# wavey-ai/soundkit

Measured on AMD Instinct MI355X. Metric: AAC-LC 1024-sample frames/s (whole node) + xrealtime, batch=4096 48 kHz stereo, higher is better.
Workload: dtype f32 (synthesis f32; s16 between the kernels as in the reference; FIR: the 16-bit samples as 2 x f16 exactly, the f32 taps as 2 x f16 to 2^-24, f32 accumulate; 1.0e-7 rel. RMS vs f64)

## Files before the change

### soundkit_amd/csrc/aac_synth.hip

```cpp
#include "sk_device.h"

#define SK_SYNTH_LOAD(p) (*(p))
#define SK_SYNTH_STORE(v, p) (*(p) = (v))

namespace sk {

namespace {

typedef float f2 __attribute__((ext_vector_type(2)));
typedef float f4 __attribute__((ext_vector_type(4)));

#ifndef SK_SYNTH_BLOCK_WAVES
#define SK_SYNTH_BLOCK_WAVES 4
#endif
constexpr int kWavesPerBlock = SK_SYNTH_BLOCK_WAVES;
#ifndef SK_WAVES_PER_SIMD
#define SK_WAVES_PER_SIMD 3
#endif
#ifndef SK_PREFETCH_DEPTH
#define SK_PREFETCH_DEPTH 1
#endif
constexpr int kDepth = SK_PREFETCH_DEPTH;
constexpr int kWavesPerSimd = SK_WAVES_PER_SIMD;
#ifndef SK_SYNTH_HOLD_ONE
#define SK_SYNTH_HOLD_ONE 1
#endif
constexpr int kExchange = 576;
constexpr int kStage = 1024;

__device__ __forceinline__ f2 cmul(f2 a, f2 b) {
    return (f2){fmaf(a.x, b.x, -a.y * b.y), fmaf(a.x, b.y, a.y * b.x)};
}
__device__ __forceinline__ f2 cadd(f2 a, f2 b) { return (f2){a.x + b.x, a.y + b.y}; }
__device__ __forceinline__ f2 csub(f2 a, f2 b) { return (f2){a.x - b.x, a.y - b.y}; }
__device__ __forceinline__ f2 mul_mi(f2 a) { return (f2){a.y, -a.x}; }

__device__ __forceinline__ void dft8(f2 (&x)[8]) {
    const float h = 0.70710678118654752440f;
    f2 t0 = cadd(x[0], x[4]), t1 = csub(x[0], x[4]);
    f2 t2 = cadd(x[2], x[6]), t3 = mul_mi(csub(x[2], x[6]));
    f2 e0 = cadd(t0, t2), e2 = csub(t0, t2), e1 = cadd(t1, t3), e3 = csub(t1, t3);
    f2 u0 = cadd(x[1], x[5]), u1 = csub(x[1], x[5]);
    f2 u2 = cadd(x[3], x[7]), u3 = mul_mi(csub(x[3], x[7]));
    f2 o0 = cadd(u0, u2), o2 = csub(u0, u2), o1 = cadd(u1, u3), o3 = csub(u1, u3);
    f2 w1 = (f2){(o1.x + o1.y) * h, (o1.y - o1.x) * h};
    f2 w2 = mul_mi(o2);
    f2 w3 = (f2){(o3.y - o3.x) * h, -(o3.x + o3.y) * h};
    x[0] = cadd(e0, o0); x[4] = csub(e0, o0);
    x[1] = cadd(e1, w1); x[5] = csub(e1, w1);
    x[2] = cadd(e2, w2); x[6] = csub(e2, w2);
    x[3] = cadd(e3, w3); x[7] = csub(e3, w3);
}

__device__ __forceinline__ void wave_sync() {
    __builtin_amdgcn_fence(__ATOMIC_ACQ_REL, "wavefront");
    __builtin_amdgcn_wave_barrier();
}

typedef const __attribute__((address_space(4))) SynthEntry *const_entries;
__device__ __forceinline__ const_entries as_constant(const SynthEntry *p) {
    return reinterpret_cast<const_entries>(reinterpret_cast<uintptr_t>(p));
}

typedef uint32_t u2 __attribute__((ext_vector_type(2)));
__device__ __forceinline__ u2 pack4_s16(const f4 &v) {
    return (u2){dev_pack2_s16(v.x, v.y), dev_pack2_s16(v.z, v.w)};
}

__device__ __forceinline__ const float *first_half_window(const float *win, int seq, int prev_shape) {
    return seq == 3 ? win + 6656 + 1024 * prev_shape : win + 2048 * prev_shape;
}
__device__ __forceinline__ const float *second_half_window(const float *win, int seq, int shape) {
    return seq == 1 ? win + 4608 + 1024 * shape : win + 2048 * shape + 1024;
}
// ... 2 lines not shown
typedef __attribute__((address_space(3))) f4 lds_f4;
typedef __attribute__((address_space(3))) float lds_f;

__device__ __forceinline__ void read_positions(const lds_f *buf, int lane, float (&v)[16]) {
#pragma unroll
    for (int r = 0; r < 2; ++r) {
        const int j = 4 * lane + 256 * r;
        const f4 f = *reinterpret_cast<const lds_f4 *>(buf + j);
        const f4 m = *reinterpret_cast<const lds_f4 *>(buf + 1020 - j);
        v[8 * r + 0] = f.x; v[8 * r + 1] = f.y; v[8 * r + 2] = f.z; v[8 * r + 3] = f.w;
        v[8 * r + 4] = m.x; v[8 * r + 5] = m.y; v[8 * r + 6] = m.z; v[8 * r + 7] = m.w;
    }
}

__device__ __forceinline__ void write_positions(lds_f *buf, int lane, const float (&v)[16]) {
#pragma unroll
    for (int r = 0; r < 2; ++r) {
        const int j = 4 * lane + 256 * r;
        *reinterpret_cast<lds_f4 *>(buf + j) = (f4){v[8 * r + 0], v[8 * r + 1], v[8 * r + 2], v[8 * r + 3]};
        *reinterpret_cast<lds_f4 *>(buf + 1020 - j) = (f4){v[8 * r + 4], v[8 * r + 5], v[8 * r + 6], v[8 * r + 7]};
    }
}

__device__ __forceinline__ void fft512(f2 (&z)[8], lds_f2 *ex, const lds_f2 *t64, f2 base2, int lane) {
    const int hi3 = lane >> 3, lo3 = lane & 7;
    dft8(z);
#pragma unroll
    for (int k = 1; k < 8; ++k) z[k] = cmul(z[k], t64[8 * k + hi3]);
#pragma unroll
    for (int k = 0; k < 8; ++k) ex[k * 68 + lane] = z[k];
    wave_sync();
#pragma unroll
    for (int n2 = 0; n2 < 8; ++n2) z[n2] = cmul(ex[lo3 * 68 + 8 * n2 + hi3], base2);
    wave_sync();
    dft8(z);
#pragma unroll
    for (int k = 1; k < 8; ++k) z[k] = cmul(z[k], t64[8 * k + hi3]);
#pragma unroll
    for (int k = 0; k < 8; ++k) ex[hi3 * 72 + k * 8 + lo3] = z[k];
    wave_sync();
#pragma unroll
    for (int n3 = 0; n3 < 8; ++n3) z[n3] = ex[n3 * 72 + lane];
    wave_sync();
    dft8(z);
}

__device__ __attribute__((noinline)) void synth_rare_frame(lds_f2 *ex, lds_f *stage, const lds_f2 *tw_lds,
                                                            const lds_f2 *t64, float base2_re, float base2_im,
                                                            const lds_f *short_win, const lds_f2 *w64, const lds_f2 *tw_short,
                                                            float *out_ptr, int16_t *out16_ptr, int seq, int prev_shape,
                                                            int shape, int lane) {
    const int hi3 = lane >> 3, lo3 = lane & 7;
    (void)base2_re, (void)base2_im, (void)t64, (void)tw_lds, (void)seq;
    const lds_f *prev_short = short_win + 256 * prev_shape;
    const lds_f *cur_short = short_win + 256 * shape;
    f2 z[8];
#pragma unroll
    for (int r = 0; r < 8; ++r) z[r] = ex[64 * r + lane];
    float dly[16];
    read_positions(stage, lane, dly);
    wave_sync();
    float o[16], d[16];

    {
#pragma unroll
        for (int w = 0; w < 8; ++w) ex[64 * w + lane] = z[w];
        wave_sync();
#pragma unroll
        for (int b2 = 0; b2 < 8; ++b2) z[b2] = ex[64 * hi3 + lo3 + 8 * b2];
        wave_sync();
        dft8(z);
#pragma unroll
        for (int kb = 1; kb < 8; ++kb) z[kb] = cmul(z[kb], w64[lo3 * kb]);
#pragma unroll
        for (int kb = 0; kb < 8; ++kb) ex[64 * hi3 + 8 * kb + lo3] = z[kb];
        wave_sync();
// ... 46 lines not shown
            if (half == 0) read_positions(stage, lane, o);
            else read_positions(stage, lane, d);
            wave_sync();
        }
    }

    float pcm[16];
#pragma unroll
    for (int i = 0; i < 16; ++i) pcm[i] = o[i] + dly[i];
    write_positions((lds_f *)ex, lane, pcm);
    write_positions(stage, lane, d);
    wave_sync();
    (void)out_ptr, (void)out16_ptr;
}

template <bool OUT16, bool ONLY_LONG>
__global__ __launch_bounds__(kWavesPerBlock * 64, (ONLY_LONG && kDepth == 1) ? kWavesPerSimd + 1 : kWavesPerSimd) void k_aac_synth(SynthArgs a) {
    __shared__ f2 lds[kWavesPerBlock][kExchange];
    __shared__ float stage_lds[ONLY_LONG ? 1 : kWavesPerBlock][ONLY_LONG ? 4 : kStage];
    __shared__ f2 tw_tab[512];
    __shared__ f2 t64_tab[64];
    __shared__ float short_win_tab[ONLY_LONG ? 2 : 512];
    __shared__ f2 short_tw_tab[ONLY_LONG ? 1 : 128];

    const int lane = threadIdx.x & 63;
    const int wave = __builtin_amdgcn_readfirstlane(threadIdx.x >> 6);
    for (int i = threadIdx.x; i < 512; i += kWavesPerBlock * 64) tw_tab[i] = reinterpret_cast<const f2 *>(a.t.tw_long)[i];
    if (threadIdx.x < 64) t64_tab[threadIdx.x] = reinterpret_cast<const f2 *>(a.t.w64)[((threadIdx.x >> 3) * (threadIdx.x & 7)) & 63];
    if (!ONLY_LONG) {
        for (int i = threadIdx.x; i < 512; i += kWavesPerBlock * 64) short_win_tab[i] = a.t.win[4096 + i];
        if (threadIdx.x < 128)
            short_tw_tab[threadIdx.x] = threadIdx.x < 64 ? reinterpret_cast<const f2 *>(a.t.w64)[threadIdx.x] : reinterpret_cast<const f2 *>(a.t.tw_short)[threadIdx.x - 64];
    }
    __syncthreads();

    const uint32_t task_id = blockIdx.x * kWavesPerBlock + wave;
    if (task_id >= a.n_tasks) return;
    lds_f2 *ex = (lds_f2 *)lds[wave];
    lds_f *stage = (lds_f *)stage_lds[ONLY_LONG ? 0 : wave];
    const lds_f2 *tw_lds = (const lds_f2 *)tw_tab;
    const lds_f2 *t64 = (const lds_f2 *)t64_tab;

    const SynthTask task_v = a.tasks[task_id];
    const uint32_t count = __builtin_amdgcn_readfirstlane(task_v.count);
    const uint32_t state = __builtin_amdgcn_readfirstlane(task_v.state);
    if (count == 0) return;
    const const_entries entries = as_constant(a.entries + __builtin_amdgcn_readfirstlane(task_v.begin));

    const int hi3 = lane >> 3, lo3 = lane & 7;
    const f2 base2 = reinterpret_cast<const f2 *>(a.t.w512)[hi3 * lo3];

    float *delay_ptr = a.delay + (size_t)state * 1024;
    int prev_shape = __builtin_amdgcn_readfirstlane((int)a.prev_shape[state]);
    float dly[16];
    {
#pragma unroll
        for (int r = 0; r < 2; ++r) {
            const int j = 4 * lane + 256 * r;
            const f4 f = *reinterpret_cast<const f4 *>(delay_ptr + j);
            const f4 m = *reinterpret_cast<const f4 *>(delay_ptr + 1020 - j);
            dly[8 * r + 0] = f.x; dly[8 * r + 1] = f.y; dly[8 * r + 2] = f.z; dly[8 * r + 3] = f.w;
            dly[8 * r + 4] = m.x; dly[8 * r + 5] = m.y; dly[8 * r + 6] = m.z; dly[8 * r + 7] = m.w;
        }
    }

    auto load_spectrum = [&](f2 (&xin)[8], uint32_t e) {
        const float *src = a.coeffs + (size_t)__builtin_amdgcn_readfirstlane(entries[e].off1024) * 1024 + 2 * lane;
#pragma unroll
        for (int r = 0; r < 8; ++r) xin[r] = SK_SYNTH_LOAD(reinterpret_cast<const f2 *>(src + 128 * r));
    };
    constexpr bool HOLD = SK_SYNTH_HOLD_ONE;
    u2 held16[HOLD && OUT16 ? 4 : 1];
    f4 held32[HOLD && !OUT16 ? 4 : 1];
// ... 7 lines not shown
                SK_SYNTH_STORE(held16[2 * r], reinterpret_cast<u2 *>(a.pcm16 + (size_t)held_off * 1024 + j));
                SK_SYNTH_STORE(held16[2 * r + 1], reinterpret_cast<u2 *>(a.pcm16 + (size_t)held_off * 1024 + 1020 - j));
            } else {
                SK_SYNTH_STORE(held32[2 * r], reinterpret_cast<f4 *>(a.pcm + (size_t)held_off * 1024 + j));
                SK_SYNTH_STORE(held32[2 * r + 1], reinterpret_cast<f4 *>(a.pcm + (size_t)held_off * 1024 + 1020 - j));
            }
        }
    };
    auto frame = [&](f2 (&xin)[8], uint32_t e) __attribute__((always_inline)) {
        const uint32_t ent_off = entries[e].off1024, ent_win = entries[e].win;
        const uint32_t win = __builtin_amdgcn_readfirstlane(ent_win);
        const int seq = (int)(win & 3);
        const int shape = (win >> 2) & 1;
        float *out_ptr = OUT16 ? nullptr : a.pcm + (size_t)__builtin_amdgcn_readfirstlane(ent_off) * 1024;
        int16_t *out16_ptr = OUT16 ? a.pcm16 + (size_t)__builtin_amdgcn_readfirstlane(ent_off) * 1024 : nullptr;

        f2 z[8];
        if (ONLY_LONG || seq != 2) {
#pragma unroll
            for (int r = 0; r < 8; ++r) {
                const float even = xin[r].x;
                const float odd = -__shfl(xin[7 - r].y, 63 - lane);
                const f2 t = tw_lds[lane + 64 * r];
                z[r] = (f2){odd * t.y - even * t.x, odd * t.x + even * t.y};
            }
        } else {
            const f2 tws = short_tw_tab[ONLY_LONG ? 0 : 64 + lane];
#pragma unroll
            for (int w = 0; w < 8; ++w) {
                const float even = xin[w].x;
                const float odd = -__shfl(xin[w].y, 63 - lane);
                z[w] = (f2){odd * tws.y - even * tws.x, odd * tws.x + even * tws.y};
            }
        }
        if (ONLY_LONG || seq != 2) {
            const float *w1 = first_half_window(a.t.win, seq, prev_shape);
            const float *w2 = second_half_window(a.t.win, seq, shape);
            f4 w1f[2], w1m[2], w2f[2], w2m[2];
#pragma unroll
            for (int r = 0; r < 2; ++r) {
                const int j = 4 * lane + 256 * r;
                w1f[r] = *reinterpret_cast<const f4 *>(w1 + j);
                w1m[r] = *reinterpret_cast<const f4 *>(w1 + 1020 - j);
                w2f[r] = *reinterpret_cast<const f4 *>(w2 + j);
                w2m[r] = *reinterpret_cast<const f4 *>(w2 + 1020 - j);
            }
            if constexpr (HOLD) {
                if (holding) store_held();
                holding = true;
                held_off = __builtin_amdgcn_readfirstlane(ent_off);
            }
            {
                const uint32_t ahead = e + kDepth < count ? e + kDepth : count - 1;
                const float *src = a.coeffs + (size_t)__builtin_amdgcn_readfirstlane(entries[ahead].off1024) * 1024 + 2 * lane;
#pragma unroll
                for (int r = 0; r < 8; ++r) xin[r] = SK_SYNTH_LOAD(reinterpret_cast<const f2 *>(src + 128 * r));
            }
            fft512(z, ex, t64, base2, lane);
#pragma unroll
            for (int j = 0; j < 8; ++j) ex[lane + 64 * j] = cmul(tw_lds[lane + 64 * j], (f2){z[j].x, -z[j].y});
            wave_sync();
#pragma unroll
            for (int r = 0; r < 2; ++r) {
                const int q = 2 * lane + 128 * r, j = 2 * q;
                const f4 F = *reinterpret_cast<const lds_f4 *>(&ex[256 + q]);
                const f4 M = *reinterpret_cast<const lds_f4 *>(&ex[254 - q]);
                const f4 W1f = w1f[r], W1m = w1m[r], W2f = w2f[r], W2m = w2m[r];
                f4 f, m;
                f.x = -F.x * W1f.x + dly[8 * r + 0]; f.y = -M.w * W1f.y + dly[8 * r + 1];
                f.z = -F.z * W1f.z + dly[8 * r + 2]; f.w = -M.y * W1f.w + dly[8 * r + 3];
                m.x = M.y * W1m.x + dly[8 * r + 4]; m.y = F.z * W1m.y + dly[8 * r + 5];
                m.z = M.w * W1m.z + dly[8 * r + 6]; m.w = F.x * W1m.w + dly[8 * r + 7];
                if constexpr (HOLD) {
                    if constexpr (OUT16) held16[2 * r] = pack4_s16(f), held16[2 * r + 1] = pack4_s16(m);
                    else held32[2 * r] = f, held32[2 * r + 1] = m;
                } else if (OUT16) {
                    SK_SYNTH_STORE(pack4_s16(f), reinterpret_cast<u2 *>(out16_ptr + j));
                    SK_SYNTH_STORE(pack4_s16(m), reinterpret_cast<u2 *>(out16_ptr + 1020 - j));
                } else {
                    SK_SYNTH_STORE(f, reinterpret_cast<f4 *>(out_ptr + j));
                    SK_SYNTH_STORE(m, reinterpret_cast<f4 *>(out_ptr + 1020 - j));
                }
                dly[8 * r + 0] = F.y * W2f.x; dly[8 * r + 1] = M.z * W2f.y;
                dly[8 * r + 2] = F.w * W2f.z; dly[8 * r + 3] = M.x * W2f.w;
                dly[8 * r + 4] = M.x * W2m.x; dly[8 * r + 5] = F.w * W2m.y;
                dly[8 * r + 6] = M.z * W2m.z; dly[8 * r + 7] = F.y * W2m.w;
            }
            wave_sync();
        } else if constexpr (!ONLY_LONG) {
            if constexpr (HOLD) {
                if (holding) store_held();
                holding = false;
            }
#pragma unroll
            for (int r = 0; r < 8; ++r) ex[64 * r + lane] = z[r];
            write_positions(stage, lane, dly);
            wave_sync();
            synth_rare_frame(ex, stage, tw_lds, t64, base2.x, base2.y, (const lds_f *)short_win_tab, (const lds_f2 *)short_tw_tab,
                             (const lds_f2 *)short_tw_tab + 64, out_ptr, out16_ptr, seq, prev_shape, shape, lane);
            read_positions(stage, lane, dly);
            float pcm[16];
            read_positions((const lds_f *)ex, lane, pcm);
            wave_sync();
            {
                const uint32_t ahead = e + kDepth < count ? e + kDepth : count - 1;
                const float *src = a.coeffs + (size_t)__builtin_amdgcn_readfirstlane(entries[ahead].off1024) * 1024 + 2 * lane;
#pragma unroll
                for (int r = 0; r < 8; ++r) xin[r] = SK_SYNTH_LOAD(reinterpret_cast<const f2 *>(src + 128 * r));
            }
#pragma unroll
            for (int r = 0; r < 2; ++r) {
                const int j = 4 * lane + 256 * r;
                const f4 f = (f4){pcm[8 * r + 0], pcm[8 * r + 1], pcm[8 * r + 2], pcm[8 * r + 3]};
                const f4 m = (f4){pcm[8 * r + 4], pcm[8 * r + 5], pcm[8 * r + 6], pcm[8 * r + 7]};
                if (OUT16) {
                    SK_SYNTH_STORE(pack4_s16(f), reinterpret_cast<u2 *>(out16_ptr + j));
                    SK_SYNTH_STORE(pack4_s16(m), reinterpret_cast<u2 *>(out16_ptr + 1020 - j));
                } else {
                    SK_SYNTH_STORE(f, reinterpret_cast<f4 *>(out_ptr + j));
                    SK_SYNTH_STORE(m, reinterpret_cast<f4 *>(out_ptr + 1020 - j));
                }
// ... 26 lines not shown
    if (lane == 0) a.prev_shape[state] = (uint8_t)prev_shape;
}

struct c2 {
    f2 re, im;
};
__device__ __forceinline__ f2 splat(float v) { return (f2){v, v}; }
__device__ __forceinline__ f2 fma2(f2 a, f2 b, f2 c) { return __builtin_elementwise_fma(a, b, c); }
__device__ __forceinline__ c2 cadd(c2 a, c2 b) { return {a.re + b.re, a.im + b.im}; }
__device__ __forceinline__ c2 csub(c2 a, c2 b) { return {a.re - b.re, a.im - b.im}; }
__device__ __forceinline__ c2 mul_mi(c2 a) { return {a.im, -a.re}; }
__device__ __forceinline__ c2 cmul_w(c2 a, f2 w) {
    const f2 wr = splat(w.x), wi = splat(w.y);
    return {fma2(a.re, wr, -(a.im * wi)), fma2(a.re, wi, a.im * wr)};
}
__device__ __forceinline__ void dft8(c2 (&x)[8]) {
    const f2 h = splat(0.70710678118654752440f);
    c2 t0 = cadd(x[0], x[4]), t1 = csub(x[0], x[4]);
    c2 t2 = cadd(x[2], x[6]), t3 = mul_mi(csub(x[2], x[6]));
    c2 e0 = cadd(t0, t2), e2 = csub(t0, t2), e1 = cadd(t1, t3), e3 = csub(t1, t3);
    c2 u0 = cadd(x[1], x[5]), u1 = csub(x[1], x[5]);
    c2 u2 = cadd(x[3], x[7]), u3 = mul_mi(csub(x[3], x[7]));
    c2 o0 = cadd(u0, u2), o2 = csub(u0, u2), o1 = cadd(u1, u3), o3 = csub(u1, u3);
    c2 w1 = {(o1.re + o1.im) * h, (o1.im - o1.re) * h};
    c2 w2 = mul_mi(o2);
    c2 w3 = {(o3.im - o3.re) * h, -((o3.re + o3.im) * h)};
    x[0] = cadd(e0, o0); x[4] = csub(e0, o0);
    x[1] = cadd(e1, w1); x[5] = csub(e1, w1);
    x[2] = cadd(e2, w2); x[6] = csub(e2, w2);
    x[3] = cadd(e3, w3); x[7] = csub(e3, w3);
}
constexpr int kPairExchange = 576;
__device__ __forceinline__ f4 as_slot(c2 v) { return (f4){v.re.x, v.re.y, v.im.x, v.im.y}; }
__device__ __forceinline__ c2 from_slot(f4 v) { return {(f2){v.x, v.y}, (f2){v.z, v.w}}; }
__device__ __forceinline__ void fft512(c2 (&z)[8], lds_f4 *ex, const lds_f2 *t64, f2 base2, int lane) {
    const int hi3 = lane >> 3, lo3 = lane & 7;
    dft8(z);
#pragma unroll
    for (int k = 1; k < 8; ++k) z[k] = cmul_w(z[k], t64[8 * k + hi3]);
#pragma unroll
    for (int k = 0; k < 8; ++k) ex[k * 66 + lane] = as_slot(z[k]);
    wave_sync();
#pragma unroll
    for (int n2 = 0; n2 < 8; ++n2) z[n2] = cmul_w(from_slot(ex[lo3 * 66 + 8 * n2 + hi3]), base2);
    wave_sync();
    dft8(z);
#pragma unroll
    for (int k = 1; k < 8; ++k) z[k] = cmul_w(z[k], t64[8 * k + hi3]);
#pragma unroll
    for (int k = 0; k < 8; ++k) ex[hi3 * 72 + k * 8 + lo3] = as_slot(z[k]);
    wave_sync();
#pragma unroll
    for (int n3 = 0; n3 < 8; ++n3) z[n3] = from_slot(ex[n3 * 72 + lane]);
    wave_sync();
    dft8(z);
}

__device__ __forceinline__ void read_positions2(const lds_f2 *buf, int lane, f2 (&v)[16]) {
#pragma unroll
    for (int r = 0; r < 2; ++r) {
        const int j = 4 * lane + 256 * r;
#pragma unroll
        for (int h = 0; h < 2; ++h) {
            const f4 f = *reinterpret_cast<const lds_f4 *>(buf + j + 2 * h);
            const f4 m = *reinterpret_cast<const lds_f4 *>(buf + 1020 - j + 2 * h);
            v[8 * r + 2 * h] = (f2){f.x, f.y}; v[8 * r + 2 * h + 1] = (f2){f.z, f.w};
            v[8 * r + 4 + 2 * h] = (f2){m.x, m.y}; v[8 * r + 4 + 2 * h + 1] = (f2){m.z, m.w};
// ... 86 lines not shown
    }
    f2 pcm[16];
#pragma unroll
    for (int i = 0; i < 16; ++i) pcm[i] = o[i] + dly[i];
    write_positions2((lds_f2 *)ex, lane, pcm);
    write_positions2(stage, lane, d);
    wave_sync();
}

template <bool OUT16, bool WITH_SHORT>
__global__ __launch_bounds__(kWavesPerBlock * 64, 2) void k_aac_synth_pair(SynthArgs a) {
    constexpr bool LDS_WIN = !WITH_SHORT;
#ifndef SK_SYNTH_HOLD_SHORT
#define SK_SYNTH_HOLD_SHORT 1
#endif
    constexpr bool HOLD = !WITH_SHORT || SK_SYNTH_HOLD_SHORT;
    __shared__ f4 lds[kWavesPerBlock][kPairExchange];
    __shared__ f4 win_tab[LDS_WIN ? 2048 : 1];
    __shared__ f2 stage_lds[WITH_SHORT ? kWavesPerBlock : 1][WITH_SHORT ? kStage : 2];
    __shared__ f2 tw_tab[512];
    __shared__ f2 t64_tab[64];
    __shared__ float short_win_tab[WITH_SHORT ? 512 : 2];
    __shared__ f2 short_tw_tab[WITH_SHORT ? 128 : 1];

    const int lane = threadIdx.x & 63;
    const int wave = __builtin_amdgcn_readfirstlane(threadIdx.x >> 6);
    for (int i = threadIdx.x; i < 512; i += kWavesPerBlock * 64) tw_tab[i] = reinterpret_cast<const f2 *>(a.t.tw_long)[i];
    if (threadIdx.x < 64) t64_tab[threadIdx.x] = reinterpret_cast<const f2 *>(a.t.w64)[((threadIdx.x >> 3) * (threadIdx.x & 7)) & 63];
    if (WITH_SHORT) {
        for (int i = threadIdx.x; i < 512; i += kWavesPerBlock * 64) short_win_tab[i] = a.t.win[4096 + i];
        if (threadIdx.x < 128)
            short_tw_tab[threadIdx.x] = threadIdx.x < 64 ? reinterpret_cast<const f2 *>(a.t.w64)[threadIdx.x] : reinterpret_cast<const f2 *>(a.t.tw_short)[threadIdx.x - 64];
    }
    if (LDS_WIN)
        for (int i = threadIdx.x; i < 2048; i += kWavesPerBlock * 64) win_tab[i] = reinterpret_cast<const f4 *>(a.t.win)[i < 1024 ? i : i + 128];
    __syncthreads();
    const lds_f *win_lds = (const lds_f *)win_tab;

    const uint32_t pair_id = blockIdx.x * kWavesPerBlock + wave;
    if (2 * pair_id + 1 >= a.n_tasks) return;
    lds_f4 *ex = (lds_f4 *)lds[wave];
    const lds_f2 *tw_lds = (const lds_f2 *)tw_tab;
    const lds_f2 *t64 = (const lds_f2 *)t64_tab;

    const SynthTask task_a = a.tasks[2 * pair_id], task_b = a.tasks[2 * pair_id + 1];
    const uint32_t count = __builtin_amdgcn_readfirstlane(task_a.count);
    if (count == 0) return;
    const uint32_t state_a = __builtin_amdgcn_readfirstlane(task_a.state), state_b = __builtin_amdgcn_readfirstlane(task_b.state);
    const const_entries ent_a = as_constant(a.entries + __builtin_amdgcn_readfirstlane(task_a.begin));
    const const_entries ent_b = as_constant(a.entries + __builtin_amdgcn_readfirstlane(task_b.begin));

    const int hi3 = lane >> 3, lo3 = lane & 7;
    const f2 base2 = reinterpret_cast<const f2 *>(a.t.w512)[hi3 * lo3];

    float *delay_a = a.delay + (size_t)state_a * 1024, *delay_b = a.delay + (size_t)state_b * 1024;
    int prev_a = __builtin_amdgcn_readfirstlane((int)a.prev_shape[state_a]);
    int prev_b = __builtin_amdgcn_readfirstlane((int)a.prev_shape[state_b]);
    float dly_a[16], dly_b[16];
    auto load_state = [&](const float *p, float (&d)[16]) {
#pragma unroll
        for (int r = 0; r < 2; ++r) {
            const int j = 4 * lane + 256 * r;
            const f4 f = *reinterpret_cast<const f4 *>(p + j);
            const f4 m = *reinterpret_cast<const f4 *>(p + 1020 - j);
            d[8 * r + 0] = f.x; d[8 * r + 1] = f.y; d[8 * r + 2] = f.z; d[8 * r + 3] = f.w;
            d[8 * r + 4] = m.x; d[8 * r + 5] = m.y; d[8 * r + 6] = m.z; d[8 * r + 7] = m.w;
        }
    };
    load_state(delay_a, dly_a);
    load_state(delay_b, dly_b);

    auto load_spectrum = [&](f2 (&xin)[8], const_entries entries, uint32_t e) {
        const float *src = a.coeffs + (size_t)__builtin_amdgcn_readfirstlane(entries[e].off1024) * 1024 + 2 * lane;
#pragma unroll
        for (int r = 0; r < 8; ++r) xin[r] = SK_SYNTH_LOAD(reinterpret_cast<const f2 *>(src + 128 * r));
    };
// ... 5 lines not shown
        const float *w2 = second_half_window(a.t.win, seq, shape);
#pragma unroll
        for (int r = 0; r < 2; ++r) {
            const int j = 4 * lane + 256 * r;
            w.w1f[r] = *reinterpret_cast<const f4 *>(w1 + j);
            w.w1m[r] = *reinterpret_cast<const f4 *>(w1 + 1020 - j);
            w.w2f[r] = *reinterpret_cast<const f4 *>(w2 + j);
            w.w2m[r] = *reinterpret_cast<const f4 *>(w2 + 1020 - j);
        }
    };
    u2 held16[HOLD && OUT16 ? 8 : 1];
    f4 held32[HOLD && !OUT16 ? 8 : 1];
    uint32_t held_off_a = 0, held_off_b = 0;
    auto emit = [&](int r, int ch, f2 F0, f2 F1, f2 M0, f2 M1, const Win &w, int w1_at, int w2_at, float (&dly)[16], float *out_ptr, int16_t *out16_ptr) {
        const int j = 4 * lane + 256 * r;
        f4 W1f, W1m, W2f, W2m;
        if constexpr (LDS_WIN) {
            W1f = *reinterpret_cast<const lds_f4 *>(win_lds + w1_at + j), W1m = *reinterpret_cast<const lds_f4 *>(win_lds + w1_at + 1020 - j);
            W2f = *reinterpret_cast<const lds_f4 *>(win_lds + w2_at + j), W2m = *reinterpret_cast<const lds_f4 *>(win_lds + w2_at + 1020 - j);
        } else {
            W1f = w.w1f[r], W1m = w.w1m[r], W2f = w.w2f[r], W2m = w.w2m[r];
        }
        f4 f, m;
        f.x = -F0.x * W1f.x + dly[8 * r + 0]; f.y = -M1.y * W1f.y + dly[8 * r + 1];
        f.z = -F1.x * W1f.z + dly[8 * r + 2]; f.w = -M0.y * W1f.w + dly[8 * r + 3];
        m.x = M0.y * W1m.x + dly[8 * r + 4]; m.y = F1.x * W1m.y + dly[8 * r + 5];
        m.z = M1.y * W1m.z + dly[8 * r + 6]; m.w = F0.x * W1m.w + dly[8 * r + 7];
        if constexpr (HOLD) {
            if constexpr (OUT16) held16[4 * r + 2 * ch] = pack4_s16(f), held16[4 * r + 2 * ch + 1] = pack4_s16(m);
            else held32[4 * r + 2 * ch] = f, held32[4 * r + 2 * ch + 1] = m;
        } else if (OUT16) {
            SK_SYNTH_STORE(pack4_s16(f), reinterpret_cast<u2 *>(out16_ptr + j));
            SK_SYNTH_STORE(pack4_s16(m), reinterpret_cast<u2 *>(out16_ptr + 1020 - j));
        } else {
            SK_SYNTH_STORE(f, reinterpret_cast<f4 *>(out_ptr + j));
            SK_SYNTH_STORE(m, reinterpret_cast<f4 *>(out_ptr + 1020 - j));
        }
        dly[8 * r + 0] = F0.y * W2f.x; dly[8 * r + 1] = M1.x * W2f.y;
        dly[8 * r + 2] = F1.y * W2f.z; dly[8 * r + 3] = M0.x * W2f.w;
        dly[8 * r + 4] = M0.x * W2m.x; dly[8 * r + 5] = F1.y * W2m.y;
        dly[8 * r + 6] = M1.x * W2m.z; dly[8 * r + 7] = F0.y * W2m.w;
    };

    lds_f2 *stage = (lds_f2 *)stage_lds[WITH_SHORT ? wave : 0];
    auto store_pcm = [&](const float (&pcm)[16], uint32_t off) __attribute__((always_inline)) {
#pragma unroll
        for (int r = 0; r < 2; ++r) {
            const int j = 4 * lane + 256 * r;
            const f4 f = (f4){pcm[8 * r + 0], pcm[8 * r + 1], pcm[8 * r + 2], pcm[8 * r + 3]};
            const f4 m = (f4){pcm[8 * r + 4], pcm[8 * r + 5], pcm[8 * r + 6], pcm[8 * r + 7]};
// ... 25 lines not shown
    };

    bool holding = false;
    f2 xa[8], xb[8];
    load_spectrum(xa, ent_a, 0);
    load_spectrum(xb, ent_b, 0);
    for (uint32_t e = 0; e < count; ++e) {
        const uint32_t off_a = __builtin_amdgcn_readfirstlane(ent_a[e].off1024), off_b = __builtin_amdgcn_readfirstlane(ent_b[e].off1024);
        const uint32_t win_a = __builtin_amdgcn_readfirstlane(ent_a[e].win), win_b = __builtin_amdgcn_readfirstlane(ent_b[e].win);
        const int shape_a = (win_a >> 2) & 1, shape_b = (win_b >> 2) & 1;
        if constexpr (WITH_SHORT) {
            if ((win_a & 3u) == 2u) {
                if constexpr (HOLD) {
                    if (holding) store_held();
                    holding = false;
                }
                {
                    const f2 tws = short_tw_tab[64 + lane];
                    const f2 tx = splat(tws.x), ty = splat(tws.y);
#pragma unroll
                    for (int w = 0; w < 8; ++w) {
                        const f2 even = (f2){xa[w].x, xb[w].x};
                        const f2 odd = (f2){-__shfl(xa[w].y, 63 - lane), -__shfl(xb[w].y, 63 - lane)};
                        const c2 zw = {odd * ty - even * tx, odd * tx + even * ty};
                        ex[64 * w + lane] = as_slot(zw);
                    }
                    f2 both[16];
#pragma unroll
                    for (int i = 0; i < 16; ++i) both[i] = (f2){dly_a[i], dly_b[i]};
                    write_positions2(stage, lane, both);
                    wave_sync();
                }
                synth_rare_pair(ex, stage, (const lds_f *)short_win_tab, (const lds_f2 *)short_tw_tab, (const lds_f2 *)short_tw_tab + 64, prev_a, shape_a, prev_b,
                                shape_b, lane);
                float pcm_a[16], pcm_b[16];
                {
                    f2 both[16];
                    read_positions2(stage, lane, both);
#pragma unroll
                    for (int i = 0; i < 16; ++i) {
                        dly_a[i] = both[i].x;
                        dly_b[i] = both[i].y;
                    }
                    read_positions2((const lds_f2 *)ex, lane, both);
#pragma unroll
                    for (int i = 0; i < 16; ++i) {
                        pcm_a[i] = both[i].x;
                        pcm_b[i] = both[i].y;
                    }
                    wave_sync();
                }
                const uint32_t ahead = e + 1 < count ? e + 1 : count - 1;
                load_spectrum(xa, ent_a, ahead);
                load_spectrum(xb, ent_b, ahead);
                store_pcm(pcm_a, off_a);
                store_pcm(pcm_b, off_b);
                prev_a = shape_a;
                prev_b = shape_b;
                continue;
            }
        }
        c2 z[8];
#pragma unroll
        for (int r = 0; r < 8; ++r) {
            const f2 even = (f2){xa[r].x, xb[r].x};
            const f2 odd = (f2){-__shfl(xa[7 - r].y, 63 - lane), -__shfl(xb[7 - r].y, 63 - lane)};
            const f2 t = tw_lds[lane + 64 * r];
            const f2 tx = splat(t.x), ty = splat(t.y);
            z[r] = {odd * ty - even * tx, odd * tx + even * ty};
        }
        Win wa, wb;
        int w1_a = 0, w2_a = 0, w1_b = 0, w2_b = 0;
        if constexpr (LDS_WIN) {
            const int seq_a = (int)(win_a & 3), seq_b = (int)(win_b & 3);
            w1_a = seq_a == 3 ? 6144 + 1024 * prev_a : 2048 * prev_a, w2_a = seq_a == 1 ? 4096 + 1024 * shape_a : 2048 * shape_a + 1024;
            w1_b = seq_b == 3 ? 6144 + 1024 * prev_b : 2048 * prev_b, w2_b = seq_b == 1 ? 4096 + 1024 * shape_b : 2048 * shape_b + 1024;
        } else {
            load_windows(wa, (int)(win_a & 3), prev_a, shape_a);
            load_windows(wb, (int)(win_b & 3), prev_b, shape_b);
        }
        if constexpr (HOLD) {
            if (holding) store_held();
            holding = true;
            held_off_a = off_a;
            held_off_b = off_b;
        }
        {
            const uint32_t ahead = e + 1 < count ? e + 1 : count - 1;
            load_spectrum(xa, ent_a, ahead);
            load_spectrum(xb, ent_b, ahead);
        }
        fft512(z, ex, t64, base2, lane);
#pragma unroll
        for (int j = 0; j < 8; ++j) {
            const f2 t = tw_lds[lane + 64 * j];
            const f2 tx = splat(t.x), ty = splat(t.y);
            const c2 v = {fma2(tx, z[j].re, -(ty * -z[j].im)), fma2(tx, -z[j].im, ty * z[j].re)};
            ex[lane + 64 * j] = as_slot(v);
        }
        wave_sync();
        float *out_a = OUT16 ? nullptr : a.pcm + (size_t)off_a * 1024, *out_b = OUT16 ? nullptr : a.pcm + (size_t)off_b * 1024;
        int16_t *out16_a = OUT16 ? a.pcm16 + (size_t)off_a * 1024 : nullptr, *out16_b = OUT16 ? a.pcm16 + (size_t)off_b * 1024 : nullptr;
#pragma unroll
        for (int r = 0; r < 2; ++r) {
            const int q = 2 * lane + 128 * r;
            const f4 F0 = ex[256 + q], F1 = ex[257 + q], M0 = ex[254 - q], M1 = ex[255 - q];
            emit(r, 0, (f2){F0.x, F0.z}, (f2){F1.x, F1.z}, (f2){M0.x, M0.z}, (f2){M1.x, M1.z}, wa, w1_a, w2_a, dly_a, out_a, out16_a);
            emit(r, 1, (f2){F0.y, F0.w}, (f2){F1.y, F1.w}, (f2){M0.y, M0.w}, (f2){M1.y, M1.w}, wb, w1_b, w2_b, dly_b, out_b, out16_b);
        }
        wave_sync();
        prev_a = shape_a;
        prev_b = shape_b;
    }
    if constexpr (HOLD) {
        if (holding) store_held();
// ... 32 lines not shown
    for (int i = threadIdx.x; i < 2 * 2 * kTailRing / 8; i += 128) reinterpret_cast<sk_u32x4 *>(&ring_lds[0][0][0])[i] = (sk_u32x4){0u, 0u, 0u, 0u};
    __syncthreads();

    const uint32_t pair_id = blockIdx.x;
    lds_f2 *ex = (lds_f2 *)lds[wave];
    const lds_f2 *tw_lds = (const lds_f2 *)tw_tab;
    const lds_f2 *t64 = (const lds_f2 *)t64_tab;
    unsigned char *ring = reinterpret_cast<unsigned char *>(&ring_lds[wave][0][0]);

    const SynthTask task_v = a.tasks[2 * pair_id + (uint32_t)wave];
    const SynthTask other_v = a.tasks[2 * pair_id + (uint32_t)(wave ^ 1)];
    const uint32_t count = __builtin_amdgcn_readfirstlane(task_v.count);
    const uint32_t state = __builtin_amdgcn_readfirstlane(task_v.state);
    const uint32_t other_state = __builtin_amdgcn_readfirstlane(other_v.state);
    if (count == 0) return;
    const const_entries entries = as_constant(a.entries + __builtin_amdgcn_readfirstlane(task_v.begin));
    const bool stereo = (state ^ other_state) == 1u;
    const uint64_t first_elem = (uint64_t)__builtin_amdgcn_readfirstlane(entries[0].off1024) * 1024u;
    const uint32_t out_row = (uint32_t)(first_elem / ta.stream_stride);
    const uint32_t n_out = (1024u * count - 130u) / 3u;
    uint32_t *dst32 = reinterpret_cast<uint32_t *>(ta.out16 + (size_t)out_row * ta.out_stride * 2);
    int16_t *dst16 = ta.out16 + (size_t)out_row * ta.out_stride;

    const int hi3 = lane >> 3, lo3 = lane & 7;
    const f2 base2 = reinterpret_cast<const f2 *>(a.t.w512)[hi3 * lo3];

    sk_u32x4 af[10][2];
    {
        const sk_u32x4 *af_src = reinterpret_cast<const sk_u32x4 *>(ta.afrag_f16) + lane;
#pragma unroll
        for (int sidx = 0; sidx < 10; ++sidx)
#pragma unroll
            for (int k = 0; k < 2; ++k) af[sidx][k] = af_src[(sidx * 2 + k) * 64];
    }

    float *delay_ptr = a.delay + (size_t)state * 1024;
    int prev_shape = __builtin_amdgcn_readfirstlane((int)a.prev_shape[state]);
    float dly[16];
#pragma unroll
    for (int r = 0; r < 2; ++r) {
        const int j = 4 * lane + 256 * r;
        const f4 f = *reinterpret_cast<const f4 *>(delay_ptr + j);
        const f4 m = *reinterpret_cast<const f4 *>(delay_ptr + 1020 - j);
        dly[8 * r + 0] = f.x; dly[8 * r + 1] = f.y; dly[8 * r + 2] = f.z; dly[8 * r + 3] = f.w;
        dly[8 * r + 4] = m.x; dly[8 * r + 5] = m.y; dly[8 * r + 6] = m.z; dly[8 * r + 7] = m.w;
    }

    auto to_ring = [&](const f4 &v, int ring_pos) __attribute__((always_inline)) {
// ... 42 lines not shown
        const uint32_t f0 = __builtin_amdgcn_perm(r2, l2, 0x05040100u), f1 = __builtin_amdgcn_perm(r2, l2, 0x07060302u);
        const uint32_t m0 = 256u * T + fm;
        if (m0 + 1 < n_out) *reinterpret_cast<u2 *>(dst32 + m0) = (u2){f0, f1};
        else if (m0 < n_out) dst32[m0] = f0;
    };

    auto load_spectrum = [&](f2 (&xin)[8], uint32_t e) {
        const float *src = a.coeffs + (size_t)__builtin_amdgcn_readfirstlane(entries[e].off1024) * 1024 + 2 * lane;
#pragma unroll
        for (int r = 0; r < 8; ++r) xin[r] = SK_SYNTH_LOAD(reinterpret_cast<const f2 *>(src + 128 * r));
    };

    uint32_t next_tile = 0;
    auto frame = [&](f2 (&xin)[8], uint32_t e) __attribute__((always_inline)) {
        const uint32_t win = __builtin_amdgcn_readfirstlane(entries[e].win);
        const int seq = (int)(win & 3);
        const int shape = (win >> 2) & 1;
        f2 z[8];
#pragma unroll
        for (int r = 0; r < 8; ++r) {
            const float even = xin[r].x;
            const float odd = -__shfl(xin[7 - r].y, 63 - lane);
            const f2 t = tw_lds[lane + 64 * r];
            z[r] = (f2){odd * t.y - even * t.x, odd * t.x + even * t.y};
        }
        const float *w1 = first_half_window(a.t.win, seq, prev_shape);
        const float *w2 = second_half_window(a.t.win, seq, shape);
        f4 w1f[2], w1m[2], w2f[2], w2m[2];
#pragma unroll
        for (int r = 0; r < 2; ++r) {
            const int j = 4 * lane + 256 * r;
            w1f[r] = *reinterpret_cast<const f4 *>(w1 + j);
            w1m[r] = *reinterpret_cast<const f4 *>(w1 + 1020 - j);
            w2f[r] = *reinterpret_cast<const f4 *>(w2 + j);
            w2m[r] = *reinterpret_cast<const f4 *>(w2 + 1020 - j);
        }
        load_spectrum(xin, e + kTailDepth < count ? e + kTailDepth : count - 1);
        fft512(z, ex, t64, base2, lane);
#pragma unroll
        for (int j = 0; j < 8; ++j) ex[lane + 64 * j] = cmul(tw_lds[lane + 64 * j], (f2){z[j].x, -z[j].y});
        wave_sync();
        const int frame_at = (int)((e & 1u) * 1024u);
#pragma unroll
        for (int r = 0; r < 2; ++r) {
            const int q = 2 * lane + 128 * r, j = 2 * q;
            const f4 F = *reinterpret_cast<const lds_f4 *>(&ex[256 + q]);
            const f4 M = *reinterpret_cast<const lds_f4 *>(&ex[254 - q]);
            const f4 W1f = w1f[r], W1m = w1m[r], W2f = w2f[r], W2m = w2m[r];
            f4 f, m;
            f.x = -F.x * W1f.x + dly[8 * r + 0]; f.y = -M.w * W1f.y + dly[8 * r + 1];
            f.z = -F.z * W1f.z + dly[8 * r + 2]; f.w = -M.y * W1f.w + dly[8 * r + 3];
            m.x = M.y * W1m.x + dly[8 * r + 4]; m.y = F.z * W1m.y + dly[8 * r + 5];
            m.z = M.w * W1m.z + dly[8 * r + 6]; m.w = F.x * W1m.w + dly[8 * r + 7];
            to_ring(f, frame_at + j);
            to_ring(m, frame_at + 1020 - j);
            dly[8 * r + 0] = F.y * W2f.x; dly[8 * r + 1] = M.z * W2f.y;
            dly[8 * r + 2] = F.w * W2f.z; dly[8 * r + 3] = M.x * W2f.w;
            dly[8 * r + 4] = M.x * W2m.x; dly[8 * r + 5] = F.w * W2m.y;
            dly[8 * r + 6] = M.z * W2m.z; dly[8 * r + 7] = F.y * W2m.w;
        }
        wave_sync();
        prev_shape = shape;
        const uint32_t have = 1024u * (e + 1);
        while (256u * next_tile < n_out && (768u * next_tile + 896u <= have || e + 1 == count)) {
            fir_tile(next_tile);
            ++next_tile;
        }
    };
    f2 ring_x[kTailDepth][8];
#pragma unroll
    for (int d = 0; d < kTailDepth; ++d) load_spectrum(ring_x[d], (uint32_t)d < count ? (uint32_t)d : count - 1);
    for (uint32_t e0 = 0; e0 < count; e0 += kTailDepth) {
#pragma unroll
        for (int d = 0; d < kTailDepth; ++d)
            if (e0 + (uint32_t)d < count) frame(ring_x[d], e0 + (uint32_t)d);
    }
// ... 139 lines not shown
```

Baseline: 271.1 million.

## Merge FFT512 stage twiddles into per-lane stage-1 table and use explicit FMAs

Restructures the 512-point FFT so the first-stage twiddles and the base2 inter-stage twiddle become one per-lane stage-1 twiddle set. This removes the complex multiply after the first LDS exchange. The set comes from a new LDS table in kernels that have spare LDS, and is preloaded into registers elsewhere. The radix-8 butterflies, pre-twiddle and windowed overlap-add are rewritten with explicit fmaf so multiply-adds are fused. The cost is extra LDS (448 f2) or 14 extra VGPRs per lane, which can lower occupancy, and a small change in rounding.

```diff
diff --git a/soundkit_amd/csrc/aac_synth.hip b/soundkit_amd/csrc/aac_synth.hip
--- a/soundkit_amd/csrc/aac_synth.hip
+++ b/soundkit_amd/csrc/aac_synth.hip
@@ -43,13 +43,15 @@
     f2 u0 = cadd(x[1], x[5]), u1 = csub(x[1], x[5]);
     f2 u2 = cadd(x[3], x[7]), u3 = mul_mi(csub(x[3], x[7]));
     f2 o0 = cadd(u0, u2), o2 = csub(u0, u2), o1 = cadd(u1, u3), o3 = csub(u1, u3);
-    f2 w1 = (f2){(o1.x + o1.y) * h, (o1.y - o1.x) * h};
+    const float s1 = o1.x + o1.y, d1 = o1.y - o1.x;
+    const float s3 = o3.x + o3.y, d3 = o3.y - o3.x;
     f2 w2 = mul_mi(o2);
-    f2 w3 = (f2){(o3.y - o3.x) * h, -(o3.x + o3.y) * h};
     x[0] = cadd(e0, o0); x[4] = csub(e0, o0);
-    x[1] = cadd(e1, w1); x[5] = csub(e1, w1);
+    x[1] = (f2){__builtin_fmaf(s1, h, e1.x), __builtin_fmaf(d1, h, e1.y)};
+    x[5] = (f2){__builtin_fmaf(-s1, h, e1.x), __builtin_fmaf(-d1, h, e1.y)};
     x[2] = cadd(e2, w2); x[6] = csub(e2, w2);
-    x[3] = cadd(e3, w3); x[7] = csub(e3, w3);
+    x[3] = (f2){__builtin_fmaf(d3, h, e3.x), __builtin_fmaf(-s3, h, e3.y)};
+    x[7] = (f2){__builtin_fmaf(-d3, h, e3.x), __builtin_fmaf(s3, h, e3.y)};
 }
 
 __device__ __forceinline__ void wave_sync() {
@@ -98,36 +100,49 @@
     }
 }
 
-__device__ __forceinline__ void fft512(f2 (&z)[8], lds_f2 *ex, const lds_f2 *t64, f2 base2, int lane) {
+constexpr int kStage1Tab = 7 * 64;
+__device__ __forceinline__ void fill_stage1_table(f2 *tab, const float2 *w512, int tid, int n_threads) {
+    for (int i = tid; i < kStage1Tab; i += n_threads) tab[i] = reinterpret_cast<const f2 *>(w512)[(i & 63) * ((i >> 6) + 1)];
+}
+__device__ __forceinline__ void stage1_twiddles(f2 (&tw1)[7], const float2 *w512, int lane) {
+#pragma unroll
+    for (int k = 1; k < 8; ++k) tw1[k - 1] = reinterpret_cast<const f2 *>(w512)[lane * k];
+}
+__device__ __forceinline__ void stage1_twiddles(f2 (&tw1)[7], const lds_f2 *tab, int lane) {
+#pragma unroll
+    for (int k = 1; k < 8; ++k) tw1[k - 1] = tab[64 * (k - 1) + lane];
+}
+
+__device__ __forceinline__ void fft512(f2 (&z)[8], lds_f2 *ex, const lds_f2 *t64, const f2 (&tw1)[7], int lane) {
     const int hi3 = lane >> 3, lo3 = lane & 7;
     dft8(z);
 #pragma unroll
+    for (int k = 1; k < 8; ++k) z[k] = cmul(z[k], tw1[k - 1]);
+#pragma unroll
+    for (int k = 0; k < 8; ++k) ex[k * 68 + lane] = z[k];
+    wave_sync();
+#pragma unroll
+    for (int n2 = 0; n2 < 8; ++n2) z[n2] = ex[lo3 * 68 + 8 * n2 + hi3];
+    wave_sync();
+    dft8(z);
+#pragma unroll
     for (int k = 1; k < 8; ++k) z[k] = cmul(z[k], t64[8 * k + hi3]);
 #pragma unroll
-    for (int k = 0; k < 8; ++k) ex[k * 68 + lane] = z[k];
-    wave_sync();
-#pragma unroll
-    for (int n2 = 0; n2 < 8; ++n2) z[n2] = cmul(ex[lo3 * 68 + 8 * n2 + hi3], base2);
+    for (int k = 0; k < 8; ++k) ex[hi3 * 72 + k * 8 + lo3] = z[k];
+    wave_sync();
+#pragma unroll
+    for (int n3 = 0; n3 < 8; ++n3) z[n3] = ex[n3 * 72 + lane];
     wave_sync();
     dft8(z);
-#pragma unroll
-    for (int k = 1; k < 8; ++k) z[k] = cmul(z[k], t64[8 * k + hi3]);
-#pragma unroll
-    for (int k = 0; k < 8; ++k) ex[hi3 * 72 + k * 8 + lo3] = z[k];
-    wave_sync();
-#pragma unroll
-    for (int n3 = 0; n3 < 8; ++n3) z[n3] = ex[n3 * 72 + lane];
-    wave_sync();
-    dft8(z);
 }
 
 __device__ __attribute__((noinline)) void synth_rare_frame(lds_f2 *ex, lds_f *stage, const lds_f2 *tw_lds,
-                                                            const lds_f2 *t64, float base2_re, float base2_im,
+                                                            const lds_f2 *t64,
                                                             const lds_f *short_win, const lds_f2 *w64, const lds_f2 *tw_short,
                                                             float *out_ptr, int16_t *out16_ptr, int seq, int prev_shape,
                                                             int shape, int lane) {
     const int hi3 = lane >> 3, lo3 = lane & 7;
-    (void)base2_re, (void)base2_im, (void)t64, (void)tw_lds, (void)seq;
+    (void)t64, (void)tw_lds, (void)seq;
     const lds_f *prev_short = short_win + 256 * prev_shape;
     const lds_f *cur_short = short_win + 256 * shape;
     f2 z[8];
@@ -220,9 +235,11 @@
     __shared__ f2 t64_tab[64];
     __shared__ float short_win_tab[ONLY_LONG ? 2 : 512];
     __shared__ f2 short_tw_tab[ONLY_LONG ? 1 : 128];
+    __shared__ f2 tw1_tab[kStage1Tab];
 
     const int lane = threadIdx.x & 63;
     const int wave = __builtin_amdgcn_readfirstlane(threadIdx.x >> 6);
+    fill_stage1_table(tw1_tab, a.t.w512, threadIdx.x, kWavesPerBlock * 64);
     for (int i = threadIdx.x; i < 512; i += kWavesPerBlock * 64) tw_tab[i] = reinterpret_cast<const f2 *>(a.t.tw_long)[i];
     if (threadIdx.x < 64) t64_tab[threadIdx.x] = reinterpret_cast<const f2 *>(a.t.w64)[((threadIdx.x >> 3) * (threadIdx.x & 7)) & 63];
     if (!ONLY_LONG) {
@@ -244,9 +261,6 @@
     const uint32_t state = __builtin_amdgcn_readfirstlane(task_v.state);
     if (count == 0) return;
     const const_entries entries = as_constant(a.entries + __builtin_amdgcn_readfirstlane(task_v.begin));
-
-    const int hi3 = lane >> 3, lo3 = lane & 7;
-    const f2 base2 = reinterpret_cast<const f2 *>(a.t.w512)[hi3 * lo3];
 
     float *delay_ptr = a.delay + (size_t)state * 1024;
     int prev_shape = __builtin_amdgcn_readfirstlane((int)a.prev_shape[state]);
@@ -300,7 +314,7 @@
                 const float even = xin[r].x;
                 const float odd = -__shfl(xin[7 - r].y, 63 - lane);
                 const f2 t = tw_lds[lane + 64 * r];
-                z[r] = (f2){odd * t.y - even * t.x, odd * t.x + even * t.y};
+                z[r] = (f2){__builtin_fmaf(odd, t.y, -(even * t.x)), __builtin_fmaf(odd, t.x, even * t.y)};
             }
         } else {
             const f2 tws = short_tw_tab[ONLY_LONG ? 0 : 64 + lane];
@@ -308,7 +322,7 @@
             for (int w = 0; w < 8; ++w) {
                 const float even = xin[w].x;
                 const float odd = -__shfl(xin[w].y, 63 - lane);
-                z[w] = (f2){odd * tws.y - even * tws.x, odd * tws.x + even * tws.y};
+                z[w] = (f2){__builtin_fmaf(odd, tws.y, -(even * tws.x)), __builtin_fmaf(odd, tws.x, even * tws.y)};
             }
         }
         if (ONLY_LONG || seq != 2) {
@@ -334,7 +348,9 @@
 #pragma unroll
                 for (int r = 0; r < 8; ++r) xin[r] = SK_SYNTH_LOAD(reinterpret_cast<const f2 *>(src + 128 * r));
             }
-            fft512(z, ex, t64, base2, lane);
+            f2 tw1[7];
+            stage1_twiddles(tw1, (const lds_f2 *)tw1_tab, lane);
+            fft512(z, ex, t64, tw1, lane);
 #pragma unroll
             for (int j = 0; j < 8; ++j) ex[lane + 64 * j] = cmul(tw_lds[lane + 64 * j], (f2){z[j].x, -z[j].y});
             wave_sync();
@@ -345,10 +361,10 @@
                 const f4 M = *reinterpret_cast<const lds_f4 *>(&ex[254 - q]);
                 const f4 W1f = w1f[r], W1m = w1m[r], W2f = w2f[r], W2m = w2m[r];
                 f4 f, m;
-                f.x = -F.x * W1f.x + dly[8 * r + 0]; f.y = -M.w * W1f.y + dly[8 * r + 1];
-                f.z = -F.z * W1f.z + dly[8 * r + 2]; f.w = -M.y * W1f.w + dly[8 * r + 3];
-                m.x = M.y * W1m.x + dly[8 * r + 4]; m.y = F.z * W1m.y + dly[8 * r + 5];
-                m.z = M.w * W1m.z + dly[8 * r + 6]; m.w = F.x * W1m.w + dly[8 * r + 7];
+                f.x = __builtin_fmaf(-F.x, W1f.x, dly[8 * r + 0]); f.y = __builtin_fmaf(-M.w, W1f.y, dly[8 * r + 1]);
+                f.z = __builtin_fmaf(-F.z, W1f.z, dly[8 * r + 2]); f.w = __builtin_fmaf(-M.y, W1f.w, dly[8 * r + 3]);
+                m.x = __builtin_fmaf(M.y, W1m.x, dly[8 * r + 4]); m.y = __builtin_fmaf(F.z, W1m.y, dly[8 * r + 5]);
+                m.z = __builtin_fmaf(M.w, W1m.z, dly[8 * r + 6]); m.w = __builtin_fmaf(F.x, W1m.w, dly[8 * r + 7]);
                 if constexpr (HOLD) {
                     if constexpr (OUT16) held16[2 * r] = pack4_s16(f), held16[2 * r + 1] = pack4_s16(m);
                     else held32[2 * r] = f, held32[2 * r + 1] = m;
@@ -374,7 +390,7 @@
             for (int r = 0; r < 8; ++r) ex[64 * r + lane] = z[r];
             write_positions(stage, lane, dly);
             wave_sync();
-            synth_rare_frame(ex, stage, tw_lds, t64, base2.x, base2.y, (const lds_f *)short_win_tab, (const lds_f2 *)short_tw_tab,
+            synth_rare_frame(ex, stage, tw_lds, t64, (const lds_f *)short_win_tab, (const lds_f2 *)short_tw_tab,
                              (const lds_f2 *)short_tw_tab + 64, out_ptr, out16_ptr, seq, prev_shape, shape, lane);
             read_positions(stage, lane, dly);
             float pcm[16];
@@ -447,27 +463,29 @@
     c2 u0 = cadd(x[1], x[5]), u1 = csub(x[1], x[5]);
     c2 u2 = cadd(x[3], x[7]), u3 = mul_mi(csub(x[3], x[7]));
     c2 o0 = cadd(u0, u2), o2 = csub(u0, u2), o1 = cadd(u1, u3), o3 = csub(u1, u3);
-    c2 w1 = {(o1.re + o1.im) * h, (o1.im - o1.re) * h};
+    const f2 s1 = o1.re + o1.im, d1 = o1.im - o1.re;
+    const f2 s3 = o3.re + o3.im, d3 = o3.im - o3.re;
     c2 w2 = mul_mi(o2);
-    c2 w3 = {(o3.im - o3.re) * h, -((o3.re + o3.im) * h)};
     x[0] = cadd(e0, o0); x[4] = csub(e0, o0);
-    x[1] = cadd(e1, w1); x[5] = csub(e1, w1);
+    x[1] = {fma2(s1, h, e1.re), fma2(d1, h, e1.im)};
+    x[5] = {fma2(-s1, h, e1.re), fma2(-d1, h, e1.im)};
     x[2] = cadd(e2, w2); x[6] = csub(e2, w2);
-    x[3] = cadd(e3, w3); x[7] = csub(e3, w3);
+    x[3] = {fma2(d3, h, e3.re), fma2(-s3, h, e3.im)};
+    x[7] = {fma2(-d3, h, e3.re), fma2(s3, h, e3.im)};
 }
 constexpr int kPairExchange = 576;
 __device__ __forceinline__ f4 as_slot(c2 v) { return (f4){v.re.x, v.re.y, v.im.x, v.im.y}; }
 __device__ __forceinline__ c2 from_slot(f4 v) { return {(f2){v.x, v.y}, (f2){v.z, v.w}}; }
-__device__ __forceinline__ void fft512(c2 (&z)[8], lds_f4 *ex, const lds_f2 *t64, f2 base2, int lane) {
+__device__ __forceinline__ void fft512(c2 (&z)[8], lds_f4 *ex, const lds_f2 *t64, const f2 (&tw1)[7], int lane) {
     const int hi3 = lane >> 3, lo3 = lane & 7;
     dft8(z);
 #pragma unroll
-    for (int k = 1; k < 8; ++k) z[k] = cmul_w(z[k], t64[8 * k + hi3]);
+    for (int k = 1; k < 8; ++k) z[k] = cmul_w(z[k], tw1[k - 1]);
 #pragma unroll
     for (int k = 0; k < 8; ++k) ex[k * 66 + lane] = as_slot(z[k]);
     wave_sync();
 #pragma unroll
-    for (int n2 = 0; n2 < 8; ++n2) z[n2] = cmul_w(from_slot(ex[lo3 * 66 + 8 * n2 + hi3]), base2);
+    for (int n2 = 0; n2 < 8; ++n2) z[n2] = from_slot(ex[lo3 * 66 + 8 * n2 + hi3]);
     wave_sync();
     dft8(z);
 #pragma unroll
@@ -600,9 +618,12 @@
     __shared__ f2 t64_tab[64];
     __shared__ float short_win_tab[WITH_SHORT ? 512 : 2];
     __shared__ f2 short_tw_tab[WITH_SHORT ? 128 : 1];
+    constexpr bool TW1_LDS = WITH_SHORT;
+    __shared__ f2 tw1_tab[TW1_LDS ? kStage1Tab : 1];
 
     const int lane = threadIdx.x & 63;
     const int wave = __builtin_amdgcn_readfirstlane(threadIdx.x >> 6);
+    if (TW1_LDS) fill_stage1_table(tw1_tab, a.t.w512, threadIdx.x, kWavesPerBlock * 64);
     for (int i = threadIdx.x; i < 512; i += kWavesPerBlock * 64) tw_tab[i] = reinterpret_cast<const f2 *>(a.t.tw_long)[i];
     if (threadIdx.x < 64) t64_tab[threadIdx.x] = reinterpret_cast<const f2 *>(a.t.w64)[((threadIdx.x >> 3) * (threadIdx.x & 7)) & 63];
     if (WITH_SHORT) {
@@ -628,8 +649,8 @@
     const const_entries ent_a = as_constant(a.entries + __builtin_amdgcn_readfirstlane(task_a.begin));
     const const_entries ent_b = as_constant(a.entries + __builtin_amdgcn_readfirstlane(task_b.begin));
 
-    const int hi3 = lane >> 3, lo3 = lane & 7;
-    const f2 base2 = reinterpret_cast<const f2 *>(a.t.w512)[hi3 * lo3];
+    f2 tw1[7];
+    if constexpr (!TW1_LDS) stage1_twiddles(tw1, a.t.w512, lane);
 
     float *delay_a = a.delay + (size_t)state_a * 1024, *delay_b = a.delay + (size_t)state_b * 1024;
     int prev_a = __builtin_amdgcn_readfirstlane((int)a.prev_shape[state_a]);
@@ -681,10 +702,14 @@
             W1f = w.w1f[r], W1m = w.w1m[r], W2f = w.w2f[r], W2m = w.w2m[r];
         }
         f4 f, m;
-        f.x = -F0.x * W1f.x + dly[8 * r + 0]; f.y = -M1.y * W1f.y + dly[8 * r + 1];
-        f.z = -F1.x * W1f.z + dly[8 * r + 2]; f.w = -M0.y * W1f.w + dly[8 * r + 3];
-        m.x = M0.y * W1m.x + dly[8 * r + 4]; m.y = F1.x * W1m.y + dly[8 * r + 5];
-        m.z = M1.y * W1m.z + dly[8 * r + 6]; m.w = F0.x * W1m.w + dly[8 * r + 7];
+        f.x = __builtin_fmaf(-F0.x, W1f.x, dly[8 * r + 0]); f.y = __builtin_fmaf(-M1.y, W1f.y, dly[8 * r + 1]);
+        f.z = __builtin_fmaf(-F1.x, W1f.z, dly[8 * r + 2]); f.w = __builtin_fmaf(-M0.y, W1f.w, dly[8 * r + 3]);
+        m.x = __builtin_fmaf(M0.y, W1m.x, dly[8 * r + 4]); m.y = __builtin_fmaf(F1.x, W1m.y, dly[8 * r + 5]);
+        m.z = __builtin_fmaf(M1.y, W1m.z, dly[8 * r + 6]); m.w = __builtin_fmaf(F0.x, W1m.w, dly[8 * r + 7]);
+        if constexpr (HOLD && !OUT16) {
+#pragma unroll
+            for (int i = 4; i < 8; ++i) __asm__ volatile("" : : "v"(m[i - 4]), "v"(dly[8 * r + i]));
+        }
         if constexpr (HOLD) {
             if constexpr (OUT16) held16[4 * r + 2 * ch] = pack4_s16(f), held16[4 * r + 2 * ch + 1] = pack4_s16(m);
             else held32[4 * r + 2 * ch] = f, held32[4 * r + 2 * ch + 1] = m;
@@ -756,7 +781,7 @@
                     for (int w = 0; w < 8; ++w) {
                         const f2 even = (f2){xa[w].x, xb[w].x};
                         const f2 odd = (f2){-__shfl(xa[w].y, 63 - lane), -__shfl(xb[w].y, 63 - lane)};
-                        const c2 zw = {odd * ty - even * tx, odd * tx + even * ty};
+                        const c2 zw = {fma2(odd, ty, -(even * tx)), fma2(odd, tx, even * ty)};
                         ex[64 * w + lane] = as_slot(zw);
                     }
                     f2 both[16];
@@ -801,7 +826,7 @@
             const f2 odd = (f2){-__shfl(xa[7 - r].y, 63 - lane), -__shfl(xb[7 - r].y, 63 - lane)};
             const f2 t = tw_lds[lane + 64 * r];
             const f2 tx = splat(t.x), ty = splat(t.y);
-            z[r] = {odd * ty - even * tx, odd * tx + even * ty};
+            z[r] = {fma2(odd, ty, -(even * tx)), fma2(odd, tx, even * ty)};
         }
         Win wa, wb;
         int w1_a = 0, w2_a = 0, w1_b = 0, w2_b = 0;
@@ -824,7 +849,8 @@
             load_spectrum(xa, ent_a, ahead);
             load_spectrum(xb, ent_b, ahead);
         }
-        fft512(z, ex, t64, base2, lane);
+        if constexpr (TW1_LDS) stage1_twiddles(tw1, (const lds_f2 *)tw1_tab, lane);
+        fft512(z, ex, t64, tw1, lane);
 #pragma unroll
         for (int j = 0; j < 8; ++j) {
             const f2 t = tw_lds[lane + 64 * j];
@@ -903,8 +929,8 @@
     uint32_t *dst32 = reinterpret_cast<uint32_t *>(ta.out16 + (size_t)out_row * ta.out_stride * 2);
     int16_t *dst16 = ta.out16 + (size_t)out_row * ta.out_stride;
 
-    const int hi3 = lane >> 3, lo3 = lane & 7;
-    const f2 base2 = reinterpret_cast<const f2 *>(a.t.w512)[hi3 * lo3];
+    f2 tw1[7];
+    stage1_twiddles(tw1, a.t.w512, lane);
 
     sk_u32x4 af[10][2];
     {
@@ -993,7 +1019,7 @@
             const float even = xin[r].x;
             const float odd = -__shfl(xin[7 - r].y, 63 - lane);
             const f2 t = tw_lds[lane + 64 * r];
-            z[r] = (f2){odd * t.y - even * t.x, odd * t.x + even * t.y};
+            z[r] = (f2){__builtin_fmaf(odd, t.y, -(even * t.x)), __builtin_fmaf(odd, t.x, even * t.y)};
         }
         const float *w1 = first_half_window(a.t.win, seq, prev_shape);
         const float *w2 = second_half_window(a.t.win, seq, shape);
@@ -1007,7 +1033,7 @@
             w2m[r] = *reinterpret_cast<const f4 *>(w2 + 1020 - j);
         }
         load_spectrum(xin, e + kTailDepth < count ? e + kTailDepth : count - 1);
-        fft512(z, ex, t64, base2, lane);
+        fft512(z, ex, t64, tw1, lane);
 #pragma unroll
         for (int j = 0; j < 8; ++j) ex[lane + 64 * j] = cmul(tw_lds[lane + 64 * j], (f2){z[j].x, -z[j].y});
         wave_sync();
@@ -1019,10 +1045,10 @@
             const f4 M = *reinterpret_cast<const lds_f4 *>(&ex[254 - q]);
             const f4 W1f = w1f[r], W1m = w1m[r], W2f = w2f[r], W2m = w2m[r];
             f4 f, m;
-            f.x = -F.x * W1f.x + dly[8 * r + 0]; f.y = -M.w * W1f.y + dly[8 * r + 1];
-            f.z = -F.z * W1f.z + dly[8 * r + 2]; f.w = -M.y * W1f.w + dly[8 * r + 3];
-            m.x = M.y * W1m.x + dly[8 * r + 4]; m.y = F.z * W1m.y + dly[8 * r + 5];
-            m.z = M.w * W1m.z + dly[8 * r + 6]; m.w = F.x * W1m.w + dly[8 * r + 7];
+            f.x = __builtin_fmaf(-F.x, W1f.x, dly[8 * r + 0]); f.y = __builtin_fmaf(-M.w, W1f.y, dly[8 * r + 1]);
+            f.z = __builtin_fmaf(-F.z, W1f.z, dly[8 * r + 2]); f.w = __builtin_fmaf(-M.y, W1f.w, dly[8 * r + 3]);
+            m.x = __builtin_fmaf(M.y, W1m.x, dly[8 * r + 4]); m.y = __builtin_fmaf(F.z, W1m.y, dly[8 * r + 5]);
+            m.z = __builtin_fmaf(M.w, W1m.z, dly[8 * r + 6]); m.w = __builtin_fmaf(F.x, W1m.w, dly[8 * r + 7]);
             to_ring(f, frame_at + j);
             to_ring(m, frame_at + 1020 - j);
             dly[8 * r + 0] = F.y * W2f.x; dly[8 * r + 1] = M.z * W2f.y;
```

After: 278.9 million (median of 6 runs). 1.03x the previous value.
